# DCASE-REPO/DESED_task

Measured on AMD Instinct MI355X. Metric: 10s-clips/sec CRNN mean-teacher train @batch48, higher is better.
Workload: dtype f32 (fp32 storage and accumulation; the dense contractions of the wide layers run as split-bf16 MFMA, 3 bf16 products per fp32 product, fp32-level accuracy; everything else exact f32)

## Files before the change

### desed_task_amd/_lib.py

```python
import ctypes
import os
import re

_HERE = os.path.dirname(os.path.abspath(__file__))
_HEADER = os.path.join(os.path.dirname(_HERE), "include", "sed_hip.h")
LIB_PATH = os.path.join(_HERE, "libsed_hip.so")

_CTYPES = {"int": ctypes.c_int, "float": ctypes.c_float, "double": ctypes.c_double, "long long": ctypes.c_longlong,
           "unsigned": ctypes.c_uint, "unsigned int": ctypes.c_uint}

ERRORS = {-1: "bad argument", -2: "kernel launch failed", -3: "unsupported configuration"}


def parse_header(path=_HEADER):
    text = open(path).read()
    text = re.sub(r"/\*.*?\*/", "", text, flags=re.S)
    protos = {}
    for m in re.finditer(r"\b(?:int|long long)\s+(sed_\w+)\s*\(([^)]*)\)\s*;", text):
        args = []
        for a in m.group(2).split(","):
            a = a.strip()
            if "*" in a:
                args.append(ctypes.c_void_p)
            else:
                ty = re.sub(r"\bconst\b", "", a).strip()
                ty = ty.rsplit(None, 1)[0].strip()
                args.append(_CTYPES[ty])
        protos[m.group(1)] = args
    return protos


def header_constants(path=_HEADER):
    return {m.group(1): int(m.group(2)) for m in re.finditer(r"^#define\s+(SED_\w+)\s+(\d+)\b", open(path).read(), re.M)}


class _Lib:
    def __init__(self, path, is_emulator=False):
        self.path = path
        self.is_emulator = is_emulator
        import torch
        self._dll = ctypes.CDLL(path)
        self.protos = parse_header()
        for name, argtypes in self.protos.items():
            fn = getattr(self._dll, name)
            fn.argtypes = argtypes
            fn.restype = ctypes.c_longlong if name.endswith("_floats") else ctypes.c_int

    def value(self, name, *args):
        return getattr(self._dll, name)(*args)

    def call(self, name, *args):
        rc = getattr(self._dll, name)(*args)
        if rc != 0:
            raise RuntimeError("%s failed: %s (rc=%d)" % (name, ERRORS.get(rc, "?"), rc))


_lib = None


def get():
    global _lib
    if _lib is None:
        if not os.path.exists(LIB_PATH):
            raise RuntimeError(
                "desed_task_amd: %s is missing -- build it with `python -m desed_task_amd.build` "
                "(hipcc --offload-arch=gfx950).  There is no CPU fallback." % LIB_PATH)
        _lib = _Lib(LIB_PATH)
    return _lib


def use_library(path, is_emulator=True):
    global _lib
    _lib = _Lib(path, is_emulator=is_emulator) if path is not None else None
    return _lib


TUNING_KEYS = {"glu_grid_cap": 0, "glu_bwd128_split": 1, "convb_ck": 2, "convb_mp": 3, "block0_nocenter": 4, "glu_fwd128": 5, "wgrad_narrow": 6, "wgrad_cap": 7, "attn_valu": 8, "wgrad_wide": 9, "gru_lds_kb": 10, "mel_taps_mem": 11, "convb_tpw": 12, "mel_wave": 13, "gemm_ntn": 14, "linear_tiles": 15}


_tuning = {}


def set_tuning(key, value):
    get().call("sed_set_tuning", TUNING_KEYS[key], int(value))
    _tuning[key] = int(value)


def get_tuning(key):
    return _tuning.get(key, 0)


def check_tensor(t, name="tensor"):
    lib = get()
    if lib.is_emulator:
        if t.is_cuda:
            raise RuntimeError("%s: emulator build bound but tensor is on the GPU" % name)
    elif not t.is_cuda:
        raise RuntimeError("%s must live on the MI355X (cuda) device: there is no CPU path" % name)
    if not t.is_contiguous():
        raise RuntimeError("%s must be contiguous" % name)


def stream_ptr(t):
    if t.is_cuda:
        import torch
        return torch.cuda.current_stream(t.device).cuda_stream
    return 0
```

### desed_task_amd/csrc/sed_common.h

```cpp
#pragma once

#ifdef SED_EMU
#include "hip_emu.h"
#else
#include <hip/hip_runtime.h>
#define SED_DYN_SMEM(name) extern __shared__ __attribute__((aligned(16))) char name[]
#define SED_LAUNCH(kern, grid, block, smem, stream, ...) \
    hipLaunchKernelGGL(kern, grid, block, smem, stream, __VA_ARGS__)
typedef float f32x16 __attribute__((ext_vector_type(16)));
typedef float f32x4 __attribute__((ext_vector_type(4)));
typedef short s16x8 __attribute__((ext_vector_type(8)));
#endif

#include <stdint.h>

#define SED_API extern "C" __attribute__((visibility("default")))

#define SED_MAX_SMEM(kern, bytes) \
    (void)hipFuncSetAttribute((const void*)(kern), hipFuncAttributeMaxDynamicSharedMemorySize, (int)(bytes))

__global__ __launch_bounds__(256) static void sed_zero4_kernel(float* p0, int n0, float* p1, int n1, float* p2, int n2, float* p3, int n3) {
    const int i = blockIdx.x * 256 + threadIdx.x;
    if (i < n0) p0[i] = 0.f;
    if (i < n1) p1[i] = 0.f;
    if (i < n2) p2[i] = 0.f;
    if (i < n3) p3[i] = 0.f;
}
static inline void sed_zero4(hipStream_t s, float* p0, int n0, float* p1, int n1, float* p2, int n2, float* p3, int n3) {
    int n = n0 > n1 ? n0 : n1;
    n = n > n2 ? n : n2;
    n = n > n3 ? n : n3;
    if (n <= 0) return;
    SED_LAUNCH(sed_zero4_kernel, dim3((n + 255) / 256), dim3(256), 0, s, p0, n0, p1, n1, p2, n2, p3, n3);
}

#define SED_OK 0
#define SED_ERR_ARG (-1)
#define SED_ERR_LAUNCH (-2)
#define SED_ERR_UNSUPPORTED (-3)

enum { SED_TUNE_GLU_GRID_CAP = 0, SED_TUNE_GLU_BWD128_SPLIT = 1, SED_TUNE_CONVB_CK = 2, SED_TUNE_CONVB_MP = 3, SED_TUNE_B0_NOCENTER = 4, SED_TUNE_GLU_FWD128 = 5, SED_TUNE_WGRAD_NARROW = 6, SED_TUNE_WGRAD_CAP = 7,
       SED_TUNE_ATTN_VALU = 8, SED_TUNE_WGRAD_WIDE = 9, SED_TUNE_GRU_LDS_KB = 10, SED_TUNE_MEL_TAPS_MEM = 11, SED_TUNE_CONVB_TPW = 12, SED_TUNE_MEL_WAVE = 13, SED_TUNE_GEMM_NTN = 14, SED_TUNE_LINEAR_TILES = 15, SED_TUNE_COUNT = 16 };
extern int sed_tuning[SED_TUNE_COUNT];

static inline int sed_check_launch() {
    hipError_t e = hipGetLastError();
    return e == hipSuccess ? SED_OK : SED_ERR_LAUNCH;
}

__device__ __forceinline__ f32x16 mfma32(float a, float b, f32x16 c) {
#ifdef SED_EMU
    return emu_mfma_32x32x2(a, b, c);
#else
    return __builtin_amdgcn_mfma_f32_32x32x2f32(a, b, c, 0, 0, 0);
#endif
}
__device__ __forceinline__ int mfma32_row(int r, int lane) { return (r & 3) + 8 * (r >> 2) + 4 * (lane >> 5); }

__device__ __forceinline__ f32x4 mfma16(float a, float b, f32x4 c) {
#ifdef SED_EMU
    return emu_mfma_16x16x4(a, b, c);
#else
    return __builtin_amdgcn_mfma_f32_16x16x4f32(a, b, c, 0, 0, 0);
#endif
}

__device__ __forceinline__ f32x16 mfma32_bf16(s16x8 a, s16x8 b, f32x16 c) {
#ifdef SED_EMU
    return emu_mfma_32x32x16_bf16(a, b, c);
#else
    typedef __bf16 bf16x8_t __attribute__((ext_vector_type(8)));
    return __builtin_amdgcn_mfma_f32_32x32x16_bf16(__builtin_bit_cast(bf16x8_t, a), __builtin_bit_cast(bf16x8_t, b), c, 0, 0, 0);
#endif
}
__device__ __forceinline__ f32x4 mfma16_bf16(s16x8 a, s16x8 b, f32x4 c) {
#ifdef SED_EMU
    return emu_mfma_16x16x32_bf16(a, b, c);
#else
    typedef __bf16 bf16x8_t __attribute__((ext_vector_type(8)));
    return __builtin_amdgcn_mfma_f32_16x16x32_bf16(__builtin_bit_cast(bf16x8_t, a), __builtin_bit_cast(bf16x8_t, b), c, 0, 0, 0);
#endif
}
__device__ __forceinline__ unsigned short f32_to_bf16(float x) {
    unsigned u = __float_as_uint(x);
    u += 0x7FFFu + ((u >> 16) & 1u);
    return (unsigned short)(u >> 16);
}
__device__ __forceinline__ float bf16_to_f32(unsigned short h) { return __uint_as_float(((unsigned)h) << 16); }
__device__ __forceinline__ void bf16_split(float x, unsigned short& hi, unsigned short& lo) {
    hi = f32_to_bf16(x);
    lo = f32_to_bf16(x - bf16_to_f32(hi));
}

__device__ __forceinline__ float sed_sadd(float a, float b) {
#ifdef SED_EMU
    return a + b;
#else
    float r;
    asm("v_add_f32 %0, %1, %2" : "=v"(r) : "v"(a), "v"(b));
    return r;
#endif
}

__device__ __forceinline__ float sed_sfma(float a, float b, float c) {
#ifdef SED_EMU
    return fmaf(a, b, c);
#else
    float r;
    asm("v_fma_f32 %0, %1, %2, %3" : "=v"(r) : "v"(a), "v"(b), "v"(c));
    return r;
#endif
}

__device__ __forceinline__ void sed_sched_fence() {
#ifndef SED_EMU
    __builtin_amdgcn_sched_barrier(0);
#endif
}

__device__ __forceinline__ unsigned sed_alignbit(unsigned hi, unsigned lo, unsigned shift) {
#ifdef SED_EMU
    return (unsigned)(((((unsigned long long)hi) << 32) | lo) >> shift);
#else
    return __builtin_amdgcn_alignbit(hi, lo, shift);
#endif
}

template <class T_>
__device__ __forceinline__ void sed_pin(T_& x) {
#ifndef SED_EMU
    asm volatile("" : "+v"(x));
#else
    (void)x;
#endif
}
__device__ __forceinline__ void sed_opaque(int& x) {
#ifndef SED_EMU
    asm volatile("" : "+v"(x));
#else
    (void)x;
#endif
}

__device__ __forceinline__ int sed_wave_uniform(int x) {
#ifdef SED_EMU
    return x;
#else
    return __builtin_amdgcn_readfirstlane(x);
#endif
}

__device__ __forceinline__ void sed_wave_sync() {
#ifdef SED_EMU
    emu_wave_sync();
#else
    __builtin_amdgcn_fence(__ATOMIC_ACQ_REL, "wavefront");
    __builtin_amdgcn_wave_barrier();
#endif
}

__device__ __forceinline__ void bf16_split2(float a, float b, unsigned& hi, unsigned& lo) {
#ifdef SED_EMU
    unsigned short h0, l0, h1, l1;
    bf16_split(a, h0, l0);
    bf16_split(b, h1, l1);
    hi = (unsigned)h0 | ((unsigned)h1 << 16);
    lo = (unsigned)l0 | ((unsigned)l1 << 16);
#else
    typedef float f32x2_t __attribute__((ext_vector_type(2)));
    typedef __bf16 bf16x2_t __attribute__((ext_vector_type(2)));
    const f32x2_t v = {a, b};
    hi = __builtin_bit_cast(unsigned, __builtin_convertvector(v, bf16x2_t));
    const f32x2_t hf = {__uint_as_float(hi << 16), __uint_as_float(hi & 0xFFFF0000u)};
    lo = __builtin_bit_cast(unsigned, __builtin_convertvector(v - hf, bf16x2_t));
#endif
}
struct SedOneProduct {};
template <class... ONE>
constexpr int sed_np() { return sizeof...(ONE) ? 1 : 3; }
__device__ __forceinline__ unsigned bf16_round2(float a, float b) {
#ifdef SED_EMU
    return (unsigned)f32_to_bf16(a) | ((unsigned)f32_to_bf16(b) << 16);
#else
    typedef float f32x2_t __attribute__((ext_vector_type(2)));
    typedef __bf16 bf16x2_t __attribute__((ext_vector_type(2)));
    const f32x2_t v = {a, b};
    return __builtin_bit_cast(unsigned, __builtin_convertvector(v, bf16x2_t));
#endif
}

__device__ __forceinline__ f32x16 f32x16_zero() {
    f32x16 z;
#pragma unroll
    for (int i = 0; i < 16; ++i) z[i] = 0.f;
    return z;
}

__device__ __forceinline__ float sed_quad_xor1(float v) {
#ifdef SED_EMU
    return __shfl_xor(v, 1);
#else
    return __builtin_bit_cast(float, __builtin_amdgcn_update_dpp(0, __builtin_bit_cast(int, v), 0xB1, 0xF, 0xF, true));
#endif
}
__device__ __forceinline__ float sed_quad_xor2(float v) {
#ifdef SED_EMU
    return __shfl_xor(v, 2);
#else
    return __builtin_bit_cast(float, __builtin_amdgcn_update_dpp(0, __builtin_bit_cast(int, v), 0x4E, 0xF, 0xF, true));
#endif
}
__device__ __forceinline__ float sed_row_ror4(float v) {
#ifdef SED_EMU
    return __shfl_xor(v, 4);
#else
    return __builtin_bit_cast(float, __builtin_amdgcn_update_dpp(0, __builtin_bit_cast(int, v), 0x124, 0xF, 0xF, true));
#endif
}
__device__ __forceinline__ float sed_row_ror8(float v) {
#ifdef SED_EMU
    return __shfl_xor(v, 8);
#else
    return __builtin_bit_cast(float, __builtin_amdgcn_update_dpp(0, __builtin_bit_cast(int, v), 0x128, 0xF, 0xF, true));
#endif
}
__device__ __forceinline__ float sed_row16_max(float v) {
    v = fmaxf(v, sed_quad_xor1(v)); v = fmaxf(v, sed_quad_xor2(v));
    v = fmaxf(v, sed_row_ror4(v)); v = fmaxf(v, sed_row_ror8(v));
    return v;
}
__device__ __forceinline__ float sed_row16_sum(float v) {
    v += sed_quad_xor1(v); v += sed_quad_xor2(v);
// ... 192 lines not shown
```

### desed_task_amd/csrc/sed_conv_bf16.hip

```cpp
#include "sed_common.h"
#include <stdlib.h>

#define CONVB_THREADS(COUT) ((COUT) >= 64 ? 512 : 256)

template <int CIN, int COUT, int TF, int MP = 128, int CKT = 32, int NP = 3>
struct ConvBCfg {
    static constexpr int PLANES = NP == 1 ? 1 : 2;
    static constexpr int TR = MP / TF;
#ifdef CONVB_OLDMAP
    static constexpr int PWL = TF + 2, PW = TF + 2, PH = TR + 2, PP = PW * PH, PPL = PWL * PH;
#else
    static constexpr int PWL = TF + 2, PW = TF == 8 ? 12 : (TF == 2 ? 6 : TF + 2), PH = TR + 2, PP = PW * PH, PPL = PWL * PH;
#endif
    static constexpr int CK = CIN < CKT ? CIN : CKT;
    static constexpr int RSS = CK + 8;
    static constexpr int NCH = CIN / CK;
    static constexpr int NT = (COUT + 31) / 32;
    static constexpr int NCOL = NT * 32;
    static constexpr int WM = MP / 32;
    static constexpr int THREADS = CONVB_THREADS(COUT);
    static constexpr int WN = THREADS / 64 / WM;
    static constexpr int NTW = NT / WN;
    static_assert(NTW >= 1 && NTW * WN == NT, "wave split must tile COUT");
    static_assert(THREADS % (CK / 4) == 0, "a thread keeps one channel quad for all its patch elements");
    static constexpr int PATCH_S = PLANES * PP * RSS;
    static constexpr int WBUF_S = PLANES * NCOL * RSS;
    static constexpr int SMEM = (PATCH_S + 3 * WBUF_S) * 2 + 64;
    static constexpr int SMEM_BNB = SMEM + 4 * CIN * 4;
    static constexpr int SLAB = PLANES * COUT * CK;
};

struct PackBJobs {
    const float* W[8];
    unsigned short* Wf[8];
    unsigned short* Wd[8];
    int cout[8], cin[8], start[9];
    int ckf[8], ckd[8];
    int n;
};
template <int PLANES = 2>
__device__ __forceinline__ void pack_weights_bf16_one(const PackBJobs& jobs, int i) {
    const int tot = jobs.start[jobs.n];
    const bool dgrad = i >= tot;
    if (dgrad) i -= tot;
    if (i >= tot) return;
    int j = 0;
#pragma unroll
    for (int q = 1; q < 8; ++q) j += (q < jobs.n && i >= jobs.start[q]) ? 1 : 0;
    if (dgrad && !jobs.Wd[j]) return;
    const int r = i - jobs.start[j], COUT = jobs.cout[j], CIN = jobs.cin[j];
    const int tap = r / (COUT * CIN), rem = r - tap * (COUT * CIN);
    unsigned short hi, lo;
    if (!dgrad) {
        const int co = rem / CIN, ci = rem - co * CIN;
        bf16_split(jobs.W[j][((size_t)co * CIN + ci) * 9 + tap], hi, lo);
        const int CK = jobs.ckf[j], NCH = CIN / CK, cc = ci / CK, cl = ci % CK;
        unsigned short* d = jobs.Wf[j] + ((size_t)(tap * NCH + cc) * PLANES * COUT + co) * CK + cl;
        d[0] = hi;
        if (PLANES == 2) d[(size_t)COUT * CK] = lo;
    } else {
        const int ci = rem / COUT, co = rem - ci * COUT;
        bf16_split(jobs.W[j][((size_t)co * CIN + ci) * 9 + (8 - tap)], hi, lo);
        const int CK = jobs.ckd[j], NCH = COUT / CK, cc = co / CK, cl = co % CK;
        unsigned short* d = jobs.Wd[j] + ((size_t)(tap * NCH + cc) * PLANES * CIN + ci) * CK + cl;
        d[0] = hi;
        if (PLANES == 2) d[(size_t)CIN * CK] = lo;
    }
}
__global__ __launch_bounds__(256) void pack_weights_bf16_kernel(PackBJobs jobs) {
    pack_weights_bf16_one(jobs, blockIdx.x * 256 + threadIdx.x);
}
__global__ __launch_bounds__(256) void pack_weights_bf16x1_kernel(PackBJobs jobs) {
    pack_weights_bf16_one<1>(jobs, blockIdx.x * 256 + threadIdx.x);
}
struct PrologueExtra {
    int* bounds; int B, nb, f_param, n_freq, t_param, n_time; uint32_t seed; const unsigned* seed_dev;
    const float4* src; float4* dst; size_t n4; const float* src_tail; float* dst_tail; int ntail;
    int pack_blocks, copy_blocks;
};
template <int PLANES>
__device__ __forceinline__ void cnn_prologue_body(const PackBJobs& jobs, const PrologueExtra& ex);
__global__ __launch_bounds__(256) void cnn_prologue_bf16x1_kernel(PackBJobs jobs, PrologueExtra ex) { cnn_prologue_body<1>(jobs, ex); }
// ... 67 lines not shown
    return sed_check_launch();
}
static int cnn_prologue_impl(bool single, int n, const void* const* W, void* const* Wf, void* const* Wd, const int* cout, const int* cin,
                            int* bounds, int B, int nb, int f_param, int n_freq, int t_param, int n_time, unsigned seed,
                            const unsigned* seed_dev, const float* copy_src, float* copy_dst, long long copy_n, void* stream) {
    if (n < 0 || n > 8) return SED_ERR_ARG;
    if (bounds && B > 0 && nb != 1 && nb != B) return SED_ERR_ARG;
    if (copy_dst && (!copy_src || copy_n < 0 || ((uintptr_t)copy_src & 15) || ((uintptr_t)copy_dst & 15))) return SED_ERR_ARG;
    PackBJobs jobs;
    const int tot = packb_jobs(jobs, n, W, Wf, Wd, cout, cin) * (packb_any_dgrad(jobs) ? 2 : 1);
    PrologueExtra ex;
    ex.bounds = (bounds && B > 0) ? bounds : nullptr; ex.B = B; ex.nb = nb; ex.f_param = f_param; ex.n_freq = n_freq;
    ex.t_param = t_param; ex.n_time = n_time; ex.seed = (uint32_t)seed; ex.seed_dev = seed_dev;
    const size_t n4 = copy_dst ? (size_t)copy_n / 4 : 0;
    ex.src = (const float4*)copy_src; ex.dst = (float4*)copy_dst; ex.n4 = n4;
    ex.ntail = copy_dst ? (int)(copy_n % 4) : 0;
    ex.src_tail = copy_src ? copy_src + 4 * n4 : nullptr; ex.dst_tail = copy_dst ? copy_dst + 4 * n4 : nullptr;
    ex.pack_blocks = (tot + 255) / 256;
    size_t cb = (n4 + 1023) / 1024;
    ex.copy_blocks = (int)(cb > 4096 ? 4096 : cb);
    if (ex.pack_blocks == 0 && !ex.bounds && n4 == 0 && ex.ntail == 0) return SED_OK;
    if (single) SED_LAUNCH(cnn_prologue_bf16x1_kernel, dim3(ex.pack_blocks + 1 + ex.copy_blocks), dim3(256), 0, (hipStream_t)stream, jobs, ex);
    else SED_LAUNCH(cnn_prologue_bf16_kernel, dim3(ex.pack_blocks + 1 + ex.copy_blocks), dim3(256), 0, (hipStream_t)stream, jobs, ex);
    return sed_check_launch();
}
SED_API int sed_cnn_prologue_bf16(int n, const void* const* W, void* const* Wf, void* const* Wd, const int* cout, const int* cin,
                                     int* bounds, int B, int nb, int f_param, int n_freq, int t_param, int n_time, unsigned seed,
                                     const unsigned* seed_dev, const float* copy_src, float* copy_dst, long long copy_n, void* stream) {
    return cnn_prologue_impl(false, n, W, Wf, Wd, cout, cin, bounds, B, nb, f_param, n_freq, t_param, n_time, seed, seed_dev, copy_src,
                             copy_dst, copy_n, stream);
}
SED_API int sed_cnn_prologue_bf16x1(int n, const void* const* W, void* const* Wf, void* const* Wd, const int* cout, const int* cin,
                                    int* bounds, int B, int nb, int f_param, int n_freq, int t_param, int n_time, unsigned seed,
                                    const unsigned* seed_dev, const float* copy_src, float* copy_dst, long long copy_n, void* stream) {
    return cnn_prologue_impl(true, n, W, Wf, Wd, cout, cin, bounds, B, nb, f_param, n_freq, t_param, n_time, seed, seed_dev, copy_src,
                             copy_dst, copy_n, stream);
}

#ifndef CONVB_ABL
#define CONVB_ABL 0
#endif

struct ConvBnb {
    const float* ybn;
    const float* stats;
    const float* gamma;
    const float* dgamma;
    const float* dbeta;
    float* dy_out;
    float* dbias;
    float inv_count;
};

template <int TF>
__device__ __forceinline__ void conv_lane_pixel(int i, int& prow, int& pcol) {
    if (TF >= 32) { prow = 0; pcol = i; return; }
#ifdef CONVB_OLDMAP
    prow = i / TF; pcol = i % TF; return;
#endif
    const int qd = i >> 2, gsel = (0x96 >> qd) & 1, g = 4 * (qd >> 1) + (i & 3);
    if (TF == 2) { prow = 8 * gsel + (g >> 1); pcol = g & 1; }
    else { prow = gsel + 2 * (g / TF); pcol = g % TF; }
}

template <int CIN, int COUT, int TF, bool STATS, int MP = 128, int CKT = 32, bool BNB = false, class... ONE>
__global__ __launch_bounds__(CONVB_THREADS(COUT)) void conv3x3_bf16_kernel(const float* __restrict__ x,
                                                                            const unsigned short* __restrict__ Wp,
                                                                            const float* __restrict__ bias, float* __restrict__ y,
                                                                            float* __restrict__ partial, int B, int T, int F,
                                                                            ConvBnb bnb) {
    constexpr int NP = sed_np<ONE...>();
    using Cfg = ConvBCfg<CIN, COUT, TF, MP, CKT, NP>;
    constexpr int TR = Cfg::TR, PW = Cfg::PW, PWL = Cfg::PWL, PP = Cfg::PP, PPL = Cfg::PPL, CK = Cfg::CK, RSS = Cfg::RSS, NCH = Cfg::NCH, NT = Cfg::NT,
                  NTW = Cfg::NTW, THREADS = Cfg::THREADS, WM = Cfg::WM, NCOL = Cfg::NCOL, SLAB = Cfg::SLAB, WBUF_S = Cfg::WBUF_S;
    SED_DYN_SMEM(smem_raw);
    unsigned short* patch = (unsigned short*)smem_raw;
    unsigned short* wbuf = patch + Cfg::PATCH_S;
    float* bnc = (float*)(smem_raw + Cfg::SMEM);
    const int tid = threadIdx.x, lane = tid & 63, w = (tid >> 6) % WM, wn = (tid >> 6) / WM, lo = lane & 31, hi = lane >> 5;
    const int ftiles = F / TF, ttiles = (T + TR - 1) / TR, ntiles = B * ttiles * ftiles;
    constexpr int WROWS = TF >= 32 ? 1 : 32 / TF;
    int lprow, lpcol;
    conv_lane_pixel<TF>(lo, lprow, lpcol);
    const int abase = (((TF >= 32 ? (32 * w) / TF : WROWS * w) + lprow) * PW + (TF >= 32 ? (32 * w) % TF : 0) + lpcol) * RSS + 8 * hi;

    f32x16 acc[NTW];

    if (NCOL > COUT) {
        for (int i = tid; i < 3 * WBUF_S; i += THREADS) wbuf[i] = 0;
        __syncthreads();
    }
    constexpr int WPIECES = SLAB / 8;
    constexpr int WV = (WPIECES + THREADS - 1) / THREADS;
    constexpr int V = CK / 4;
    constexpr int NLD = (PPL * V + THREADS - 1) / THREADS;
    uint4 wreg[3 * WV];
    float4 ld[NLD];
    float4 ldy[BNB ? NLD : 1];
    if (BNB) {
        for (int c = tid; c < CIN; c += THREADS) {
            const float g = bnb.gamma[c];
            bnc[c] = bnb.stats[c];
            bnc[CIN + c] = bnb.stats[CIN + c];
            bnc[2 * CIN + c] = g * bnb.dbeta[c] * bnb.inv_count;
            bnc[3 * CIN + c] = g * bnb.dgamma[c] * bnb.inv_count;
        }
        if (blockIdx.x == 0 && tid < CIN && bnb.dbias != nullptr) bnb.dbias[tid] = 0.f;
        __syncthreads();
    }
    auto w_dst = [&](int buf, int piece) -> unsigned short* {
        const int plane = piece / (COUT * CK / 8), rem = piece - plane * (COUT * CK / 8);
        const int co = rem / (CK / 8), pc = rem - co * (CK / 8);
        return wbuf + buf * WBUF_S + plane * NCOL * RSS + co * RSS + 8 * pc;
    };
    auto load_row = [&](int cc, int r) {
#pragma unroll
        for (int t3 = 0; t3 < 3; ++t3) {
            const uint4* src = (const uint4*)(Wp + ((size_t)(3 * r + t3) * NCH + cc) * SLAB);
#pragma unroll
            for (int i = 0; i < WV; ++i) {
                const int piece = tid + THREADS * i;
                uint4 v = make_uint4(0u, 0u, 0u, 0u);
                if (piece < WPIECES && !(CONVB_ABL & 1)) v = src[piece];
                wreg[t3 * WV + i] = v;
            }
        }
    };
    auto store_row = [&]() {
#pragma unroll
        for (int t3 = 0; t3 < 3; ++t3)
#pragma unroll
            for (int i = 0; i < WV; ++i) {
                const int piece = tid + THREADS * i;
                if (piece < WPIECES) *(uint4*)w_dst(t3, piece) = wreg[t3 * WV + i];
            }
    };
    auto load_patch = [&](int cc, int pb, int pt0, int pf0) {
#pragma unroll
        for (int u = 0; u < NLD; ++u) {
            const int idx = tid + THREADS * u;
            const int pix = idx / V, v = idx - pix * V;
            const int i = pix / PWL, j = pix - i * PWL;
            const int t = pt0 - 1 + i, f = pf0 - 1 + j;
            ld[u] = make_float4(0.f, 0.f, 0.f, 0.f);
            if (BNB) ldy[u] = make_float4(0.f, 0.f, 0.f, 0.f);
            if (idx < PPL * V && t >= 0 && t < T && f >= 0 && f < F && !(CONVB_ABL & 4)) {
                const size_t off = (((size_t)pb * T + t) * F + f) * CIN + cc * CK + 4 * v;
                ld[u] = *(const float4*)(x + off);
                if (BNB) ldy[u] = *(const float4*)(bnb.ybn + off);
            }
        }
    };
    constexpr bool PERS = CIN <= 32;
    bool primed = false;
    int tile_it = blockIdx.x;
    do {
    const int tile = PERS ? tile_it : (int)blockIdx.x;
    const int ft = tile % ftiles, tt = (tile / ftiles) % ttiles, b = tile / (ftiles * ttiles);
    const int t0 = tt * TR, f0 = ft * TF;
    const int tile_n = PERS ? tile + (int)gridDim.x : ntiles;
    int nb = 0, nt0 = 0, nf0 = 0;
    if (PERS && tile_n < ntiles) { nb = tile_n / (ftiles * ttiles); nt0 = ((tile_n / ftiles) % ttiles) * TR; nf0 = (tile_n % ftiles) * TF; }
    auto store_patch = [&](int cc) {
        float4 bmean, bistd, bm1, bm2;
        if (BNB) {
            const int c0 = cc * CK + 4 * (tid % V);
            bmean = *(const float4*)(bnc + c0);
            bistd = *(const float4*)(bnc + CIN + c0);
            bm1 = *(const float4*)(bnc + 2 * CIN + c0);
            bm2 = *(const float4*)(bnc + 3 * CIN + c0);
        }
#pragma unroll
        for (int u = 0; u < NLD; ++u) {
            const int idx = tid + THREADS * u;
            if (idx < PPL * V) {
                const int pixl = idx / V, v = idx - pixl * V;
                const int i = pixl / PWL, j = pixl - i * PWL, pix = i * PW + j;
                if (BNB) {
                    const int t = t0 - 1 + i, f = f0 - 1 + j;
                    if (t >= 0 && t < T && f >= 0 && f < F) {
                        float4 g = ld[u];
                        const float4 yv = ldy[u];
                        g.x = bistd.x * (g.x - bm1.x - (yv.x - bmean.x) * bistd.x * bm2.x);
                        g.y = bistd.y * (g.y - bm1.y - (yv.y - bmean.y) * bistd.y * bm2.y);
                        g.z = bistd.z * (g.z - bm1.z - (yv.z - bmean.z) * bistd.z * bm2.z);
                        g.w = bistd.w * (g.w - bm1.w - (yv.w - bmean.w) * bistd.w * bm2.w);
                        ld[u] = g;
                        if (i >= 1 && i <= TR && j >= 1 && j <= TF)
                            *(float4*)(bnb.dy_out + (((size_t)b * T + t) * F + f) * CIN + cc * CK + 4 * v) = g;
                    }
                }
                if constexpr (NP == 1) {
                    *(uint2*)(patch + pix * RSS + 4 * v) = make_uint2(bf16_round2(ld[u].x, ld[u].y), bf16_round2(ld[u].z, ld[u].w));
                } else {
                uint2 hv, lv;
                bf16_split2(ld[u].x, ld[u].y, hv.x, lv.x);
                bf16_split2(ld[u].z, ld[u].w, hv.y, lv.y);
                *(uint2*)(patch + pix * RSS + 4 * v) = hv;
                *(uint2*)(patch + PP * RSS + pix * RSS + 4 * v) = lv;
                }
            }
        }
    };

#pragma unroll
    for (int nt = 0; nt < NTW; ++nt) acc[nt] = f32x16_zero();
    if (!PERS || !primed) {
        load_patch(0, b, t0, f0);
        load_row(0, 0);
        primed = true;
    }
    store_patch(0);
    store_row();
    __syncthreads();
#pragma unroll 1
    for (int cc = 0; cc < NCH; ++cc) {
#pragma unroll
        for (int r = 0; r < 3; ++r) {
            const bool next_chunk = r == 2 && cc + 1 < NCH;
            const bool more = r < 2 || cc + 1 < NCH;
            if (more) load_row(r < 2 ? cc : cc + 1, r < 2 ? r + 1 : 0);
            if (next_chunk) load_patch(cc + 1, b, t0, f0);
            if (PERS && !more && tile_n < ntiles) {
                load_row(0, 0);
                load_patch(0, nb, nt0, nf0);
            }
#pragma unroll
            for (int t3 = 0; t3 < 3; ++t3) {
                const unsigned short* wb = wbuf + t3 * WBUF_S;
                const unsigned short* ap = patch + abase + (r * PW + t3) * RSS;
#pragma unroll
                for (int ks = 0; ks < CK / 16; ++ks) {
                    if constexpr (NP == 1) {
                        const s16x8 a1 = *(const s16x8*)(ap + 16 * ks);
#pragma unroll
                        for (int nt = 0; nt < NTW; ++nt)
                            acc[nt] = mfma32_bf16(a1, *(const s16x8*)(wb + ((wn * NTW + nt) * 32 + lo) * RSS + 16 * ks + 8 * hi), acc[nt]);
                        continue;
                    }
                    s16x8 a_hi, a_lo;
                    if (CONVB_ABL & 16) { a_hi = (s16x8)(short)(lane + ks); a_lo = (s16x8)(short)(lane + t3); }
                    else { a_hi = *(const s16x8*)(ap + 16 * ks); a_lo = *(const s16x8*)(ap + PP * RSS + 16 * ks); }
#pragma unroll
                    for (int nt = 0; nt < NTW; ++nt) {
                        const unsigned short* bp = wb + ((wn * NTW + nt) * 32 + lo) * RSS + 16 * ks + 8 * hi;
                        s16x8 b_hi, b_lo;
                        if (CONVB_ABL & 16) { b_hi = (s16x8)(short)(lane + nt); b_lo = (s16x8)(short)(lane + r); }
                        else { b_hi = *(const s16x8*)bp; b_lo = *(const s16x8*)(bp + NCOL * RSS); }
                        if (CONVB_ABL & 2) { acc[nt][0] += (float)(a_lo[0] + b_hi[0] + a_hi[1] + b_lo[1]); continue; }
                        acc[nt] = mfma32_bf16(a_lo, b_hi, acc[nt]);
                        acc[nt] = mfma32_bf16(a_hi, b_lo, acc[nt]);
                        acc[nt] = mfma32_bf16(a_hi, b_hi, acc[nt]);
                    }
                }
            }
            if (!(CONVB_ABL & 8)) __syncthreads();
            if (more) store_row();
            if (next_chunk) store_patch(cc + 1);
            if (!(CONVB_ABL & 8)) __syncthreads();
        }
    }
    float* red = (float*)wbuf;
#pragma unroll
    for (int nt = 0; nt < NTW; ++nt) {
        const int co = (wn * NTW + nt) * 32 + lo;
        const float bv = (bias != nullptr && co < COUT) ? bias[co] : 0.f;
        float s = 0.f, s2 = 0.f;
#pragma unroll
        for (int r = 0; r < 16; ++r) {
            int eprow, epcol;
            conv_lane_pixel<TF>(mfma32_row(r, lane), eprow, epcol);
            const int t = t0 + (TF >= 32 ? (32 * w) / TF : WROWS * w) + eprow, f = f0 + (TF >= 32 ? (32 * w) % TF : 0) + epcol;
            if (t < T && co < COUT) {
                const float v = acc[nt][r] + bv;
                if (!(CONVB_ABL & 32)) y[(((size_t)b * T + t) * F + f) * COUT + co] = v;
                s += v;
                s2 += v * v;
            }
        }
        if (STATS) {
            s += __shfl_xor(s, 32);
            s2 += __shfl_xor(s2, 32);
            if (hi == 0) {
                red[(w * 2 + 0) * (NT * 32) + co] = s;
                red[(w * 2 + 1) * (NT * 32) + co] = s2;
            }
        }
    }
    if (STATS) {
        __syncthreads();
        if (tid < 2 * COUT) {
            const int which = tid / COUT, co = tid - which * COUT;
            float v = 0.f;
#pragma unroll
            for (int ww = 0; ww < WM; ++ww) v += red[(ww * 2 + which) * (NT * 32) + co];
            partial[(size_t)tid * ntiles + tile] = v;
        }
    }
    if (PERS && STATS && NCOL > COUT) {
        __syncthreads();
        for (int i = tid; i < 3 * WBUF_S; i += THREADS) wbuf[i] = 0;
    }
    if constexpr (!PERS) break;
    __syncthreads();
    tile_it += (int)gridDim.x;
    } while (tile_it < ntiles);
}

template <class K>
static inline int convb_persistent_grid(K kern, int threads, int smem, int ntiles, int CIN) {
    if (CIN > 32) return ntiles;
    const int e = sed_tuning[SED_TUNE_CONVB_TPW];
    if (e < 0) return ntiles;
    if (e > 0) return (ntiles + e - 1) / e;
#ifdef SED_EMU
    (void)kern; (void)threads; (void)smem;
    return ntiles;
#else
    static int slots = 0;
    if (slots == 0) {
        int per_cu = 0, dev = 0;
        hipDeviceProp_t prop;
        if (hipGetDevice(&dev) != hipSuccess || hipGetDeviceProperties(&prop, dev) != hipSuccess ||
            hipOccupancyMaxActiveBlocksPerMultiprocessor(&per_cu, (const void*)kern, threads, (size_t)smem) != hipSuccess || per_cu < 1)
            slots = -1;
        else
            slots = per_cu * prop.multiProcessorCount;
    }
    if (slots < 0 || ntiles <= 2 * slots) return ntiles;
    return slots;
#endif
}

template <int CIN, int COUT, int TF, bool STATS, int MP, int CKT, bool BNB, int NP>
struct ConvKern {
    static constexpr auto fn = NP == 1 ? conv3x3_bf16_kernel<CIN, COUT, TF, STATS, MP, CKT, BNB, SedOneProduct> : conv3x3_bf16_kernel<CIN, COUT, TF, STATS, MP, CKT, BNB>;
};
template <int CIN, int COUT, int TF, int MP = 128, int CKT = 32, bool BNB = false, int NP = 3>
static int launch_convb(const float* x, const unsigned short* Wp, const float* bias, float* y, float* partial, int B, int T, int F,
                        hipStream_t s, ConvBnb bnb = ConvBnb()) {
    using Cfg = ConvBCfg<CIN, COUT, TF, MP, CKT, NP>;
    const int ntiles = B * ((T + Cfg::TR - 1) / Cfg::TR) * (F / TF);
    if constexpr (BNB) {
        if constexpr (CIN >= COUT) {
            SED_MAX_SMEM((ConvKern<CIN, COUT, TF, false, MP, CKT, true, NP>::fn), Cfg::SMEM_BNB);
            const int nblk = convb_persistent_grid(ConvKern<CIN, COUT, TF, false, MP, CKT, true, NP>::fn, Cfg::THREADS, Cfg::SMEM_BNB, ntiles, CIN);
            SED_LAUNCH((ConvKern<CIN, COUT, TF, false, MP, CKT, true, NP>::fn), dim3(nblk), dim3(Cfg::THREADS), Cfg::SMEM_BNB, s, x, Wp, bias, y, partial, B, T, F, bnb);
            return sed_check_launch();
        } else {
            return SED_ERR_UNSUPPORTED;
        }
    } else if (partial) {
        SED_MAX_SMEM((ConvKern<CIN, COUT, TF, true, MP, CKT, false, NP>::fn), Cfg::SMEM);
        const int nblk = convb_persistent_grid(ConvKern<CIN, COUT, TF, true, MP, CKT, false, NP>::fn, Cfg::THREADS, Cfg::SMEM, ntiles, CIN);
        SED_LAUNCH((ConvKern<CIN, COUT, TF, true, MP, CKT, false, NP>::fn), dim3(nblk), dim3(Cfg::THREADS), Cfg::SMEM, s, x, Wp, bias, y, partial, B, T, F, bnb);
    } else {
        SED_MAX_SMEM((ConvKern<CIN, COUT, TF, false, MP, CKT, false, NP>::fn), Cfg::SMEM);
        const int nblk = convb_persistent_grid(ConvKern<CIN, COUT, TF, false, MP, CKT, false, NP>::fn, Cfg::THREADS, Cfg::SMEM, ntiles, CIN);
        SED_LAUNCH((ConvKern<CIN, COUT, TF, false, MP, CKT, false, NP>::fn), dim3(nblk), dim3(Cfg::THREADS), Cfg::SMEM, s, x, Wp, bias, y, partial, B, T, F, bnb);
    }
    return sed_check_launch();
}

static inline int convb_mp(int F, int CIN, int COUT) {
    const int e = sed_tuning[SED_TUNE_CONVB_MP];
    if (e && COUT >= 64) return e;
    if (COUT < 64) return 128;
    if (CIN <= 32) return 128;
    if (CIN == 128 && COUT == 128 && F <= 2) return 64;
    if (CIN == 128 && COUT == 128 && F <= 4) return 128;
    return 256;
}
SED_API int sed_conv_fwd_blocks_bf16(int B, int T, int F, int CIN, int COUT) {
    if (CIN == 1) return B * ((T + 15) / 16);
    const int TF = F >= 32 ? 32 : F;
    const int TR = convb_mp(F, CIN, COUT) / TF;
    return B * ((T + TR - 1) / TR) * (F / TF);
}

template <bool BNB, int NP = 3>
static int convb_dispatch(const float* x, const void* Wp, const float* bias, float* y, float* partial, int B, int T, int F,
                          int CIN, int COUT, hipStream_t s, ConvBnb bnb) {
    if (B <= 0 || T <= 0) return SED_OK;
    const int TF = F >= 32 ? 32 : F;
    if (F % TF != 0 || (F & (F - 1)) != 0 || F < 2) return SED_ERR_UNSUPPORTED;
    const unsigned short* W = (const unsigned short*)Wp;
    const int MP = convb_mp(F, CIN, COUT);
    const int CK = CIN >= 32 ? convb_ck(CIN, COUT) : 32;
#define CONVB_CASE16(ci, co, tf, mp) \
    if (CIN == ci && COUT == co && TF == tf && MP == mp && CK == 16) return launch_convb<ci, co, tf, mp, 16, BNB, NP>(x, W, bias, y, partial, B, T, F, s, bnb);
    CONVB_CASE16(32, 64, 32, 128) CONVB_CASE16(64, 128, 16, 128) CONVB_CASE16(64, 128, 16, 256)
    CONVB_CASE16(128, 128, 8, 128) CONVB_CASE16(128, 128, 8, 256) CONVB_CASE16(128, 128, 4, 64) CONVB_CASE16(128, 128, 4, 128)
    CONVB_CASE16(128, 128, 2, 64) CONVB_CASE16(128, 128, 2, 128) CONVB_CASE16(64, 32, 32, 128)
    CONVB_CASE16(128, 64, 16, 128) CONVB_CASE16(128, 64, 16, 256)
    CONVB_CASE16(64, 128, 4, 256) CONVB_CASE16(64, 128, 8, 256) CONVB_CASE16(64, 128, 32, 256)
    CONVB_CASE16(128, 64, 4, 256) CONVB_CASE16(128, 64, 8, 256) CONVB_CASE16(128, 64, 32, 256)
#undef CONVB_CASE16
    if (CK == 16) return SED_ERR_UNSUPPORTED;
#define CONVB_CASE(ci, co, tf, mp) \
    if (CIN == ci && COUT == co && TF == tf && MP == mp) return launch_convb<ci, co, tf, mp, 32, BNB, NP>(x, W, bias, y, partial, B, T, F, s, bnb);
    CONVB_CASE(16, 32, 32, 128)
    CONVB_CASE(32, 64, 32, 128) CONVB_CASE(32, 64, 32, 256)
    CONVB_CASE(64, 128, 16, 128) CONVB_CASE(64, 128, 16, 256)
    CONVB_CASE(128, 128, 8, 128) CONVB_CASE(128, 128, 8, 256)
    CONVB_CASE(128, 128, 4, 64) CONVB_CASE(128, 128, 4, 128) CONVB_CASE(128, 128, 4, 256)
    CONVB_CASE(128, 128, 2, 64) CONVB_CASE(128, 128, 2, 128)
    CONVB_CASE(32, 16, 32, 128) CONVB_CASE(64, 32, 32, 128)
    CONVB_CASE(128, 64, 16, 128) CONVB_CASE(128, 64, 16, 256)
    CONVB_CASE(16, 32, 16, 128) CONVB_CASE(32, 64, 8, 256) CONVB_CASE(32, 64, 16, 256) CONVB_CASE(64, 128, 4, 256) CONVB_CASE(64, 128, 8, 256)
    CONVB_CASE(64, 128, 32, 256) CONVB_CASE(128, 128, 16, 256) CONVB_CASE(128, 128, 32, 256)
    CONVB_CASE(32, 16, 16, 128) CONVB_CASE(64, 32, 8, 128) CONVB_CASE(64, 32, 16, 128) CONVB_CASE(128, 64, 4, 256) CONVB_CASE(128, 64, 8, 256)
    CONVB_CASE(128, 64, 32, 256)
#undef CONVB_CASE
    return SED_ERR_UNSUPPORTED;
}

SED_API int sed_conv3x3_bf16x3(const float* x, const void* Wp, const float* bias, float* y, float* partial, int B, int T, int F,
                                  int CIN, int COUT, void* stream) {
    return convb_dispatch<false>(x, Wp, bias, y, partial, B, T, F, CIN, COUT, (hipStream_t)stream, ConvBnb());
}

SED_API int sed_conv3x3_bf16x3_bnbwd(const float* dz, const float* ybn, const float* stats, const float* gamma, const float* dgamma,
                                        const float* dbeta, const void* Wd, float* dx, float* dy_out, float* dbias, int B, int T, int F,
                                        int CIN, int COUT, void* stream) {
    if (!dz || !ybn || !stats || !gamma || !dgamma || !dbeta || !dy_out || dy_out == dz) return SED_ERR_ARG;
    ConvBnb bnb;
    bnb.ybn = ybn; bnb.stats = stats; bnb.gamma = gamma; bnb.dgamma = dgamma; bnb.dbeta = dbeta; bnb.dy_out = dy_out; bnb.dbias = dbias;
    bnb.inv_count = 1.0f / (float)((size_t)B * T * F);
    return convb_dispatch<true>(dz, Wd, nullptr, dx, nullptr, B, T, F, CIN, COUT, (hipStream_t)stream, bnb);
}

SED_API int sed_conv3x3_bf16x1(const float* x, const void* Wp, const float* bias, float* y, float* partial, int B, int T, int F,
                               int CIN, int COUT, void* stream) {
    return convb_dispatch<false, 1>(x, Wp, bias, y, partial, B, T, F, CIN, COUT, (hipStream_t)stream, ConvBnb());
}
SED_API int sed_conv3x3_bf16x1_bnbwd(const float* dz, const float* ybn, const float* stats, const float* gamma, const float* dgamma,
                                     const float* dbeta, const void* Wd, float* dx, float* dy_out, float* dbias, int B, int T, int F,
                                     int CIN, int COUT, void* stream) {
    if (!dz || !ybn || !stats || !gamma || !dgamma || !dbeta || !dy_out || dy_out == dz) return SED_ERR_ARG;
    ConvBnb bnb;
    bnb.ybn = ybn; bnb.stats = stats; bnb.gamma = gamma; bnb.dgamma = dgamma; bnb.dbeta = dbeta; bnb.dy_out = dy_out; bnb.dbias = dbias;
    bnb.inv_count = 1.0f / (float)((size_t)B * T * F);
    return convb_dispatch<true, 1>(dz, Wd, nullptr, dx, nullptr, B, T, F, CIN, COUT, (hipStream_t)stream, bnb);
}
```

Before: 16580.

## Add double-buffered weight-row pipeline for deep 128x128 conv layers

Adds a pipelined variant of the bf16 3x3 conv kernel for the 128->128 layers at small frequency tiles (TF 4 and 2). It double-buffers the weight rows in LDS and registers, prefetching two rows ahead, and fully unrolls the row loop so global loads overlap the MFMA work. The variant launches one block per tile instead of using the persistent grid. It is on by default because the tuning flag defaults to 0. In exchange it doubles the weight LDS footprint and register use, which may lower occupancy. It also uses scalar-laundered global pointers and bounds the zero-padding handling of the patch load.

Result: no change. 16640, median of 6 (+0.4%).

```diff
diff --git a/desed_task_amd/_lib.py b/desed_task_amd/_lib.py
--- a/desed_task_amd/_lib.py
+++ b/desed_task_amd/_lib.py
@@ -75,7 +75,7 @@
     return _lib
 
 
-TUNING_KEYS = {"glu_grid_cap": 0, "glu_bwd128_split": 1, "convb_ck": 2, "convb_mp": 3, "block0_nocenter": 4, "glu_fwd128": 5, "wgrad_narrow": 6, "wgrad_cap": 7, "attn_valu": 8, "wgrad_wide": 9, "gru_lds_kb": 10, "mel_taps_mem": 11, "convb_tpw": 12, "mel_wave": 13, "gemm_ntn": 14, "linear_tiles": 15}
+TUNING_KEYS = {"glu_grid_cap": 0, "glu_bwd128_split": 1, "convb_ck": 2, "convb_mp": 3, "block0_nocenter": 4, "glu_fwd128": 5, "wgrad_narrow": 6, "wgrad_cap": 7, "attn_valu": 8, "wgrad_wide": 9, "gru_lds_kb": 10, "mel_taps_mem": 11, "convb_tpw": 12, "mel_wave": 13, "gemm_ntn": 14, "linear_tiles": 15, "convb_pipe": 16}
 
 
 _tuning = {}
diff --git a/desed_task_amd/csrc/sed_common.h b/desed_task_amd/csrc/sed_common.h
--- a/desed_task_amd/csrc/sed_common.h
+++ b/desed_task_amd/csrc/sed_common.h
@@ -40,7 +40,7 @@
 #define SED_ERR_UNSUPPORTED (-3)
 
 enum { SED_TUNE_GLU_GRID_CAP = 0, SED_TUNE_GLU_BWD128_SPLIT = 1, SED_TUNE_CONVB_CK = 2, SED_TUNE_CONVB_MP = 3, SED_TUNE_B0_NOCENTER = 4, SED_TUNE_GLU_FWD128 = 5, SED_TUNE_WGRAD_NARROW = 6, SED_TUNE_WGRAD_CAP = 7,
-       SED_TUNE_ATTN_VALU = 8, SED_TUNE_WGRAD_WIDE = 9, SED_TUNE_GRU_LDS_KB = 10, SED_TUNE_MEL_TAPS_MEM = 11, SED_TUNE_CONVB_TPW = 12, SED_TUNE_MEL_WAVE = 13, SED_TUNE_GEMM_NTN = 14, SED_TUNE_LINEAR_TILES = 15, SED_TUNE_COUNT = 16 };
+       SED_TUNE_ATTN_VALU = 8, SED_TUNE_WGRAD_WIDE = 9, SED_TUNE_GRU_LDS_KB = 10, SED_TUNE_MEL_TAPS_MEM = 11, SED_TUNE_CONVB_TPW = 12, SED_TUNE_MEL_WAVE = 13, SED_TUNE_GEMM_NTN = 14, SED_TUNE_LINEAR_TILES = 15, SED_TUNE_CONVB_PIPE = 16, SED_TUNE_COUNT = 17 };
 extern int sed_tuning[SED_TUNE_COUNT];
 
 static inline int sed_check_launch() {
@@ -132,6 +132,22 @@
     asm volatile("" : "+v"(x));
 #else
     (void)x;
+#endif
+}
+template <class T_>
+__device__ __forceinline__ void sed_launder(const T_*& p) {
+#ifndef SED_EMU
+    asm volatile("" : "+s"(p));
+#else
+    (void)p;
+#endif
+}
+__device__ __forceinline__ float4 sed_global_load4(const float* p) {
+#ifndef SED_EMU
+    const f32x4 v = *(const __attribute__((address_space(1))) f32x4*)p;
+    return make_float4(v[0], v[1], v[2], v[3]);
+#else
+    return *(const float4*)p;
 #endif
 }
 __device__ __forceinline__ void sed_opaque(int& x) {
@@ -176,8 +192,12 @@
 #endif
 }
 struct SedOneProduct {};
+template <class A_, class B_> struct sed_same { static constexpr bool value = false; };
+template <class A_> struct sed_same<A_, A_> { static constexpr bool value = true; };
+template <class M_, class... ONE>
+constexpr bool sed_has_marker() { return (false || ... || sed_same<M_, ONE>::value); }
 template <class... ONE>
-constexpr int sed_np() { return sizeof...(ONE) ? 1 : 3; }
+constexpr int sed_np() { return sed_has_marker<SedOneProduct, ONE...>() ? 1 : 3; }
 __device__ __forceinline__ unsigned bf16_round2(float a, float b) {
 #ifdef SED_EMU
     return (unsigned)f32_to_bf16(a) | ((unsigned)f32_to_bf16(b) << 16);
diff --git a/desed_task_amd/csrc/sed_conv_bf16.hip b/desed_task_amd/csrc/sed_conv_bf16.hip
--- a/desed_task_amd/csrc/sed_conv_bf16.hip
+++ b/desed_task_amd/csrc/sed_conv_bf16.hip
@@ -28,6 +28,8 @@
     static constexpr int SMEM = (PATCH_S + 3 * WBUF_S) * 2 + 64;
     static constexpr int SMEM_BNB = SMEM + 4 * CIN * 4;
     static constexpr int SLAB = PLANES * COUT * CK;
+    static constexpr int SMEM_PIPE = (PATCH_S + 2 * 3 * WBUF_S) * 2 + 64;
+    static constexpr int SMEM_PIPE_BNB = SMEM_PIPE + 4 * CIN * 4;
 };
 
 struct PackBJobs {
@@ -201,6 +203,8 @@
     float inv_count;
 };
 
+struct SedPipe {};
+
 template <int TF>
 __device__ __forceinline__ void conv_lane_pixel(int i, int& prow, int& pcol) {
     if (TF >= 32) { prow = 0; pcol = i; return; }
@@ -219,13 +223,16 @@
                                                                             float* __restrict__ partial, int B, int T, int F,
                                                                             ConvBnb bnb) {
     constexpr int NP = sed_np<ONE...>();
+    constexpr bool PIPE = sed_has_marker<SedPipe, ONE...>();
     using Cfg = ConvBCfg<CIN, COUT, TF, MP, CKT, NP>;
+    static_assert(!PIPE || (CIN > 32 && Cfg::NCOL == COUT), "SedPipe: multi-chunk layers with whole MFMA tiles of outputs only");
+    static_assert(!PIPE || Cfg::SMEM_PIPE_BNB <= 160 * 1024, "SedPipe: patch + two weight rows must fit the CU's 160 KB of LDS");
     constexpr int TR = Cfg::TR, PW = Cfg::PW, PWL = Cfg::PWL, PP = Cfg::PP, PPL = Cfg::PPL, CK = Cfg::CK, RSS = Cfg::RSS, NCH = Cfg::NCH, NT = Cfg::NT,
                   NTW = Cfg::NTW, THREADS = Cfg::THREADS, WM = Cfg::WM, NCOL = Cfg::NCOL, SLAB = Cfg::SLAB, WBUF_S = Cfg::WBUF_S;
     SED_DYN_SMEM(smem_raw);
     unsigned short* patch = (unsigned short*)smem_raw;
     unsigned short* wbuf = patch + Cfg::PATCH_S;
-    float* bnc = (float*)(smem_raw + Cfg::SMEM);
+    float* bnc = (float*)(smem_raw + (PIPE ? Cfg::SMEM_PIPE : Cfg::SMEM));
     const int tid = threadIdx.x, lane = tid & 63, w = (tid >> 6) % WM, wn = (tid >> 6) / WM, lo = lane & 31, hi = lane >> 5;
     const int ftiles = F / TF, ttiles = (T + TR - 1) / TR, ntiles = B * ttiles * ftiles;
     constexpr int WROWS = TF >= 32 ? 1 : 32 / TF;
@@ -244,6 +251,7 @@
     constexpr int V = CK / 4;
     constexpr int NLD = (PPL * V + THREADS - 1) / THREADS;
     uint4 wreg[3 * WV];
+    uint4 wreg2[PIPE ? 3 * WV : 1];
     float4 ld[NLD];
     float4 ldy[BNB ? NLD : 1];
     if (BNB) {
@@ -282,6 +290,30 @@
             for (int i = 0; i < WV; ++i) {
                 const int piece = tid + THREADS * i;
                 if (piece < WPIECES) *(uint4*)w_dst(t3, piece) = wreg[t3 * WV + i];
+            }
+    };
+    static_assert(!PIPE || WPIECES % THREADS == 0, "SedPipe: every thread moves the same number of 16-byte pieces");
+    auto load_row_p = [&](int i, bool odd) {
+        const int cc = i / 3, r = i - 3 * cc;
+#pragma unroll
+        for (int t3 = 0; t3 < 3; ++t3) {
+            const uint4* src = (const uint4*)(Wp + ((size_t)(3 * r + t3) * NCH + cc) * SLAB);
+#pragma unroll
+            for (int k = 0; k < WV; ++k) {
+                const int piece = tid + THREADS * k;
+                uint4 v = make_uint4(0u, 0u, 0u, 0u);
+                if (!(CONVB_ABL & 1)) v = src[piece];
+                if (odd) wreg2[t3 * WV + k] = v; else wreg[t3 * WV + k] = v;
+            }
+        }
+    };
+    auto store_row_p = [&](bool odd) {
+#pragma unroll
+        for (int t3 = 0; t3 < 3; ++t3)
+#pragma unroll
+            for (int k = 0; k < WV; ++k) {
+                const int piece = tid + THREADS * k;
+                *(uint4*)w_dst((odd ? 3 : 0) + t3, piece) = odd ? wreg2[t3 * WV + k] : wreg[t3 * WV + k];
             }
     };
     auto load_patch = [&](int cc, int pb, int pt0, int pf0) {
@@ -298,6 +330,22 @@
                 ld[u] = *(const float4*)(x + off);
                 if (BNB) ldy[u] = *(const float4*)(bnb.ybn + off);
             }
+        }
+    };
+    const float* xl = x;
+    const float* yl = bnb.ybn;
+    if constexpr (PIPE) { sed_launder(xl); sed_launder(yl); }
+    auto load_patch_p = [&](int cc, int pb, int pt0, int pf0) {
+#pragma unroll
+        for (int u = 0; u < NLD; ++u) {
+            const int idx = tid + THREADS * u;
+            const int pix = idx / V, v = idx - pix * V;
+            const int i = pix / PWL, j = pix - i * PWL;
+            const int t = pt0 - 1 + i, f = pf0 - 1 + j;
+            const bool ok = idx < PPL * V && t >= 0 && t < T && f >= 0 && f < F;
+            const size_t off = (((size_t)pb * T + (ok ? t : pt0)) * F + (ok ? f : pf0)) * CIN + cc * CK + 4 * v;
+            ld[u] = sed_global_load4(xl + off);
+            if (BNB) ldy[u] = sed_global_load4(yl + off);
         }
     };
     constexpr bool PERS = CIN <= 32;
@@ -325,6 +373,10 @@
             if (idx < PPL * V) {
                 const int pixl = idx / V, v = idx - pixl * V;
                 const int i = pixl / PWL, j = pixl - i * PWL, pix = i * PW + j;
+                if constexpr (PIPE) {
+                    const int t = t0 - 1 + i, f = f0 - 1 + j;
+                    if (!(t >= 0 && t < T && f >= 0 && f < F) || (CONVB_ABL & 4)) ld[u] = make_float4(0.f, 0.f, 0.f, 0.f);
+                }
                 if (BNB) {
                     const int t = t0 - 1 + i, f = f0 - 1 + j;
                     if (t >= 0 && t < T && f >= 0 && f < F) {
@@ -354,39 +406,19 @@
 
 #pragma unroll
     for (int nt = 0; nt < NTW; ++nt) acc[nt] = f32x16_zero();
-    if (!PERS || !primed) {
-        load_patch(0, b, t0, f0);
-        load_row(0, 0);
-        primed = true;
-    }
-    store_patch(0);
-    store_row();
-    __syncthreads();
-#pragma unroll 1
-    for (int cc = 0; cc < NCH; ++cc) {
-#pragma unroll
-        for (int r = 0; r < 3; ++r) {
-            const bool next_chunk = r == 2 && cc + 1 < NCH;
-            const bool more = r < 2 || cc + 1 < NCH;
-            if (more) load_row(r < 2 ? cc : cc + 1, r < 2 ? r + 1 : 0);
-            if (next_chunk) load_patch(cc + 1, b, t0, f0);
-            if (PERS && !more && tile_n < ntiles) {
-                load_row(0, 0);
-                load_patch(0, nb, nt0, nf0);
-            }
-#pragma unroll
-            for (int t3 = 0; t3 < 3; ++t3) {
-                const unsigned short* wb = wbuf + t3 * WBUF_S;
-                const unsigned short* ap = patch + abase + (r * PW + t3) * RSS;
-#pragma unroll
-                for (int ks = 0; ks < CK / 16; ++ks) {
-                    if constexpr (NP == 1) {
-                        const s16x8 a1 = *(const s16x8*)(ap + 16 * ks);
-#pragma unroll
-                        for (int nt = 0; nt < NTW; ++nt)
-                            acc[nt] = mfma32_bf16(a1, *(const s16x8*)(wb + ((wn * NTW + nt) * 32 + lo) * RSS + 16 * ks + 8 * hi), acc[nt]);
-                        continue;
-                    }
+    auto mfma_row = [&](int r, const unsigned short* wb0) {
+#pragma unroll
+        for (int t3 = 0; t3 < 3; ++t3) {
+            const unsigned short* wb = wb0 + t3 * WBUF_S;
+            const unsigned short* ap = patch + abase + (r * PW + t3) * RSS;
+#pragma unroll
+            for (int ks = 0; ks < CK / 16; ++ks) {
+                if constexpr (NP == 1) {
+                    const s16x8 a1 = *(const s16x8*)(ap + 16 * ks);
+#pragma unroll
+                    for (int nt = 0; nt < NTW; ++nt)
+                        acc[nt] = mfma32_bf16(a1, *(const s16x8*)(wb + ((wn * NTW + nt) * 32 + lo) * RSS + 16 * ks + 8 * hi), acc[nt]);
+                } else {
                     s16x8 a_hi, a_lo;
                     if (CONVB_ABL & 16) { a_hi = (s16x8)(short)(lane + ks); a_lo = (s16x8)(short)(lane + t3); }
                     else { a_hi = *(const s16x8*)(ap + 16 * ks); a_lo = *(const s16x8*)(ap + PP * RSS + 16 * ks); }
@@ -403,11 +435,90 @@
                     }
                 }
             }
+        }
+    };
+    if constexpr (PIPE) {
+        constexpr int NROW = 3 * NCH;
+        load_patch_p(0, b, t0, f0);
+        load_row_p(0, false);
+        sed_sched_fence();
+        load_row_p(1, true);
+        sed_sched_fence();
+        store_patch(0);
+        store_row_p(false);
+        __syncthreads();
+#pragma unroll
+        for (int i = 0; i < NROW; ++i) {
+            const int cc = i / 3, r = i - 3 * cc;
+            const bool odd = i & 1;
+            if (i + 2 < NROW) load_row_p(i + 2, odd);
+            if (r == 0 && cc + 1 < NCH) load_patch_p(cc + 1, b, t0, f0);
+            sed_sched_fence();
+            mfma_row(r, wbuf + (odd ? 3 : 0) * WBUF_S);
+            sed_sched_fence();
+            if (i + 1 < NROW) store_row_p(!odd);
+            if (!(CONVB_ABL & 8)) __syncthreads();
+            if (r == 2 && cc + 1 < NCH) {
+                store_patch(cc + 1);
+                if (!(CONVB_ABL & 8)) __syncthreads();
+            }
+        }
+    } else {
+    if (!PERS || !primed) {
+        load_patch(0, b, t0, f0);
+        load_row(0, 0);
+        primed = true;
+    }
+    store_patch(0);
+    store_row();
+    __syncthreads();
+#pragma unroll 1
+    for (int cc = 0; cc < NCH; ++cc) {
+#pragma unroll
+        for (int r = 0; r < 3; ++r) {
+            const bool next_chunk = r == 2 && cc + 1 < NCH;
+            const bool more = r < 2 || cc + 1 < NCH;
+            if (more) load_row(r < 2 ? cc : cc + 1, r < 2 ? r + 1 : 0);
+            if (next_chunk) load_patch(cc + 1, b, t0, f0);
+            if (PERS && !more && tile_n < ntiles) {
+                load_row(0, 0);
+                load_patch(0, nb, nt0, nf0);
+            }
+#pragma unroll
+            for (int t3 = 0; t3 < 3; ++t3) {
+                const unsigned short* wb = wbuf + t3 * WBUF_S;
+                const unsigned short* ap = patch + abase + (r * PW + t3) * RSS;
+#pragma unroll
+                for (int ks = 0; ks < CK / 16; ++ks) {
+                    if constexpr (NP == 1) {
+                        const s16x8 a1 = *(const s16x8*)(ap + 16 * ks);
+#pragma unroll
+                        for (int nt = 0; nt < NTW; ++nt)
+                            acc[nt] = mfma32_bf16(a1, *(const s16x8*)(wb + ((wn * NTW + nt) * 32 + lo) * RSS + 16 * ks + 8 * hi), acc[nt]);
+                        continue;
+                    }
+                    s16x8 a_hi, a_lo;
+                    if (CONVB_ABL & 16) { a_hi = (s16x8)(short)(lane + ks); a_lo = (s16x8)(short)(lane + t3); }
+                    else { a_hi = *(const s16x8*)(ap + 16 * ks); a_lo = *(const s16x8*)(ap + PP * RSS + 16 * ks); }
+#pragma unroll
+                    for (int nt = 0; nt < NTW; ++nt) {
+                        const unsigned short* bp = wb + ((wn * NTW + nt) * 32 + lo) * RSS + 16 * ks + 8 * hi;
+                        s16x8 b_hi, b_lo;
+                        if (CONVB_ABL & 16) { b_hi = (s16x8)(short)(lane + nt); b_lo = (s16x8)(short)(lane + r); }
+                        else { b_hi = *(const s16x8*)bp; b_lo = *(const s16x8*)(bp + NCOL * RSS); }
+                        if (CONVB_ABL & 2) { acc[nt][0] += (float)(a_lo[0] + b_hi[0] + a_hi[1] + b_lo[1]); continue; }
+                        acc[nt] = mfma32_bf16(a_lo, b_hi, acc[nt]);
+                        acc[nt] = mfma32_bf16(a_hi, b_lo, acc[nt]);
+                        acc[nt] = mfma32_bf16(a_hi, b_hi, acc[nt]);
+                    }
+                }
+            }
             if (!(CONVB_ABL & 8)) __syncthreads();
             if (more) store_row();
             if (next_chunk) store_patch(cc + 1);
             if (!(CONVB_ABL & 8)) __syncthreads();
         }
+    }
     }
     float* red = (float*)wbuf;
 #pragma unroll
@@ -485,6 +596,26 @@
 struct ConvKern {
     static constexpr auto fn = NP == 1 ? conv3x3_bf16_kernel<CIN, COUT, TF, STATS, MP, CKT, BNB, SedOneProduct> : conv3x3_bf16_kernel<CIN, COUT, TF, STATS, MP, CKT, BNB>;
 };
+template <int CIN, int COUT, int TF, bool STATS, int MP, bool BNB, int NP>
+struct ConvKernPipe {
+    static constexpr auto fn = NP == 1 ? conv3x3_bf16_kernel<CIN, COUT, TF, STATS, MP, 32, BNB, SedOneProduct, SedPipe> : conv3x3_bf16_kernel<CIN, COUT, TF, STATS, MP, 32, BNB, SedPipe>;
+};
+template <int CIN, int COUT, int TF, int MP, bool BNB, int NP>
+static int launch_convb_pipe(const float* x, const unsigned short* Wp, const float* bias, float* y, float* partial, int B, int T, int F,
+                             hipStream_t s, ConvBnb bnb) {
+    using Cfg = ConvBCfg<CIN, COUT, TF, MP, 32, NP>;
+    const int ntiles = B * ((T + Cfg::TR - 1) / Cfg::TR) * (F / TF);
+    if constexpr (BNB) {
+        SED_MAX_SMEM((ConvKernPipe<CIN, COUT, TF, false, MP, true, NP>::fn), Cfg::SMEM_PIPE_BNB);
+        SED_LAUNCH((ConvKernPipe<CIN, COUT, TF, false, MP, true, NP>::fn), dim3(ntiles), dim3(Cfg::THREADS), Cfg::SMEM_PIPE_BNB, s, x, Wp, bias, y, partial, B, T, F, bnb);
+    } else if (partial) {
+        SED_MAX_SMEM((ConvKernPipe<CIN, COUT, TF, true, MP, false, NP>::fn), Cfg::SMEM_PIPE);
+        SED_LAUNCH((ConvKernPipe<CIN, COUT, TF, true, MP, false, NP>::fn), dim3(ntiles), dim3(Cfg::THREADS), Cfg::SMEM_PIPE, s, x, Wp, bias, y, partial, B, T, F, bnb);
+    } else {
+        return SED_ERR_UNSUPPORTED;
+    }
+    return sed_check_launch();
+}
 template <int CIN, int COUT, int TF, int MP = 128, int CKT = 32, bool BNB = false, int NP = 3>
 static int launch_convb(const float* x, const unsigned short* Wp, const float* bias, float* y, float* partial, int B, int T, int F,
                         hipStream_t s, ConvBnb bnb = ConvBnb()) {
@@ -546,6 +677,10 @@
     CONVB_CASE16(128, 64, 4, 256) CONVB_CASE16(128, 64, 8, 256) CONVB_CASE16(128, 64, 32, 256)
 #undef CONVB_CASE16
     if (CK == 16) return SED_ERR_UNSUPPORTED;
+    if (CIN == 128 && COUT == 128 && (BNB || partial) && !sed_tuning[SED_TUNE_CONVB_PIPE]) {
+        if (TF == 4 && MP == 128) return launch_convb_pipe<128, 128, 4, 128, BNB, NP>(x, W, bias, y, partial, B, T, F, s, bnb);
+        if (TF == 2 && MP == 64) return launch_convb_pipe<128, 128, 2, 64, BNB, NP>(x, W, bias, y, partial, B, T, F, s, bnb);
+    }
 #define CONVB_CASE(ci, co, tf, mp) \
     if (CIN == ci && COUT == co && TF == tf && MP == mp) return launch_convb<ci, co, tf, mp, 32, BNB, NP>(x, W, bias, y, partial, B, T, F, s, bnb);
     CONVB_CASE(16, 32, 32, 128)
```
